# FordyceLab/magnify

Hardware: AMD Instinct MI355X
Metric: megapixels/sec through flatfield+segment+ROI-reduce; markers/sec (higher is better)
Workload: dtype u16

## Files before the change

magnify_amd/csrc/mg_edges.hip:

```cpp
#include <math.h>
#include <stdlib.h>

#include <algorithm>

#include "mg_common.h"

namespace {

constexpr int TW = 256;
constexpr int TH = 64;
constexpr int NT = 256;
constexpr int RPW = 16;
constexpr int LPAD = 16;
constexpr int LS = TW + 2 * LPAD;
constexpr int CHUNKS = LS / 16;

struct U8Scale {
  double mn, top, scale, offset;
  int passthrough;
};

__device__ __forceinline__ U8Scale make_scale(const double* d_minmax, int plane) {
  U8Scale s;
  s.passthrough = (d_minmax == nullptr);
// ... 551 lines not shown
}

__device__ __forceinline__ int nth_window(const int32_t* coarse, int p) {
  int last = -1;
  for (int it = 0; it <= p; ++it) {
    int best = 0x7FFFFFFF;
#pragma unroll
    for (int k = 0; k < 4; ++k)
      if (coarse[k] > last && coarse[k] < best) best = coarse[k];
    if (best == 0x7FFFFFFF) return -1;
    last = best;
  }
  return last;
}

__device__ __forceinline__ long long block_exscan_i64(long long mine, long long* s_pre) {
  s_pre[threadIdx.x] = mine;
  __syncthreads();
  for (int off = 1; off < NT; off <<= 1) {
    const long long v = (int)threadIdx.x >= off ? s_pre[threadIdx.x - off] : 0;
    __syncthreads();
    s_pre[threadIdx.x] += v;
    __syncthreads();
  }
  return s_pre[threadIdx.x] - mine;
}

__global__ __launch_bounds__(NT) void k_edge_thresholds(const uint32_t* __restrict__ d_hist, int n_fine, int n_bins,
                                                        long long r0, long long r1, long long r2, long long r3,
                                                        float gamma_lo, float gamma_hi, int32_t* __restrict__ d_thresh,
                                                        float* __restrict__ d_quantiles, int32_t* __restrict__ d_unresolved,
                                                        int32_t* __restrict__ d_state, uint32_t* __restrict__ d_win_base) {
  __shared__ int s_bin[4];
  __shared__ long long s_below[4];
  __shared__ uint32_t s_hist[FINE + COARSE];
  const int plane = blockIdx.x;
  const uint32_t* hist_g = d_hist + (int64_t)plane * n_bins;
  for (int i = threadIdx.x; i < n_bins; i += NT) s_hist[i] = hist_g[i];
  __syncthreads();
  const uint32_t* hist = s_hist;
  const int per = (n_bins + NT - 1) / NT;
  const int b0 = threadIdx.x * per, b1 = min(b0 + per, n_bins);
  long long mine = 0;
  for (int b = b0; b < b1; ++b) mine += hist[b];
  __shared__ long long s_pre[NT];
  long long run = block_exscan_i64(mine, s_pre);
  if (threadIdx.x < 4) s_bin[threadIdx.x] = n_bins, s_below[threadIdx.x] = 0;
  __syncthreads();
  const long long ranks[4] = {r0, r1, r2, r3};
  for (int b = b0; b < b1; ++b) {
    const long long nxt = run + hist[b];
#pragma unroll
    for (int k = 0; k < 4; ++k)
      if (run <= ranks[k] && ranks[k] < nxt) s_bin[k] = b, s_below[k] = run;
    run = nxt;
  }
  __syncthreads();
  if (threadIdx.x == 0) {
    int32_t order[4], coarse[4];
#pragma unroll
    for (int k = 0; k < 4; ++k) {
      const bool fine = s_bin[k] < n_fine || s_bin[k] >= n_bins;
      order[k] = fine ? s_bin[k] : 0;
      coarse[k] = fine ? -1 : s_bin[k] - n_fine;
    }
    int n_win = 0;
    while (nth_window(coarse, n_win) >= 0) ++n_win;
    d_unresolved[plane] = n_win | (n_win << 8);
    if (d_state) {
      int32_t* st = d_state + (int64_t)plane * TS_WORDS;
#pragma unroll
      for (int k = 0; k < 4; ++k) {
        st[TS_ORDER + k] = order[k];
        st[TS_COARSE + k] = coarse[k];
        st[TS_RESID + k] = (int32_t)(ranks[k] - s_below[k]);
      }
      st[TS_NWIN] = n_win;
    }
    if (d_win_base) d_win_base[plane] = n_win > 0 ? (uint32_t)nth_window(coarse, 0) << 13 : MG_HIST_SKIP;
    finish_thresholds(order, gamma_lo, gamma_hi, plane, d_thresh, d_quantiles);
  }
}

__global__ __launch_bounds__(NT) void k_window_resolve(const uint32_t* __restrict__ d_hist_win, int pass, float gamma_lo,
                                                       float gamma_hi, int32_t* __restrict__ d_state,
                                                       uint32_t* __restrict__ d_win_base, int32_t* __restrict__ d_thresh,
                                                       float* __restrict__ d_quantiles, int32_t* __restrict__ d_unresolved) {
  __shared__ int s_pos[4];
  __shared__ long long s_pre[NT];
  const int plane = blockIdx.x;
  int32_t* st = d_state + (int64_t)plane * TS_WORDS;
  const int n_win = st[TS_NWIN];
  if (pass >= n_win) return;
  int32_t coarse[4], resid[4];
#pragma unroll
  for (int k = 0; k < 4; ++k) coarse[k] = st[TS_COARSE + k], resid[k] = st[TS_RESID + k];
  const int cbin = nth_window(coarse, pass);
  const uint32_t* hist = d_hist_win + (int64_t)plane * FINE;
  constexpr int PER = FINE / NT;
  uint32_t mine_v[PER];
  long long mine = 0;
#pragma unroll
  for (int j = 0; j < PER; ++j) mine_v[j] = hist[threadIdx.x * PER + j], mine += mine_v[j];
  long long run = block_exscan_i64(mine, s_pre);
  if (threadIdx.x < 4) s_pos[threadIdx.x] = 0;
  __syncthreads();
#pragma unroll
  for (int j = 0; j < PER; ++j) {
    const long long nxt = run + mine_v[j];
#pragma unroll
    for (int k = 0; k < 4; ++k)
      if (coarse[k] == cbin && run <= (long long)resid[k] && (long long)resid[k] < nxt) s_pos[k] = threadIdx.x * PER + j;
    run = nxt;
  }
  __syncthreads();
  if (threadIdx.x == 0) {
    int32_t order[4];
#pragma unroll
    for (int k = 0; k < 4; ++k) {
      order[k] = st[TS_ORDER + k];
      if (coarse[k] == cbin) order[k] = (cbin << 13) + s_pos[k], st[TS_ORDER + k] = order[k];
    }
    const int left = n_win - 1 - pass;
    d_unresolved[plane] = left | (n_win << 8);
    d_win_base[plane] = left > 0 ? (uint32_t)nth_window(coarse, pass + 1) << 13 : MG_HIST_SKIP;
    if (left == 0) finish_thresholds(order, gamma_lo, gamma_hi, plane, d_thresh, d_quantiles);
  }
}

__device__ __forceinline__ uint32_t bits_at(const uint32_t* __restrict__ bits, int64_t bit0, int n) {
  const int64_t wi = bit0 >> 5;
  const int sh = (int)(bit0 & 31);
  uint64_t two = bits[wi];
  if (sh + n > 32) two |= (uint64_t)bits[wi + 1] << 32;
  const uint32_t v = (uint32_t)(two >> sh);
  return n >= 32 ? v : (v & ((1u << n) - 1u));
}
__device__ __forceinline__ void bits_or(uint32_t* __restrict__ bits, int64_t bit0, uint32_t v) {
  if (!v) return;
  const int64_t wi = bit0 >> 5;
  const int sh = (int)(bit0 & 31);
  atomicOr(&bits[wi], v << sh);
  if (sh && (v >> (32 - sh))) atomicOr(&bits[wi + 1], v >> (32 - sh));
}
__device__ __forceinline__ uint32_t row_word(const uint32_t* __restrict__ bits, int h, int w, int y, int x0) {
  if (y < 0 || y >= h) return 0u;
  const int lo = max(x0, 0), hi = min(x0 + 32, w);
  if (lo >= hi) return 0u;
  return bits_at(bits, (int64_t)y * w + lo, hi - lo) << (lo - x0);
}

__device__ __forceinline__ uint32_t shl1_or(uint32_t v, uint64_t mask) {
  uint32_t out;
  uint64_t carry_out;
  asm("v_addc_co_u32_e64 %0, %1, %2, %2, %3" : "=v"(out), "=s"(carry_out) : "v"(v), "s"(mask));
  return out;
}

__device__ __forceinline__ uint32_t or_reduce8(uint32_t v) {
  v |= (uint32_t)__builtin_amdgcn_update_dpp(0, (int)v, 0xB1, 0xF, 0xF, true);
  v |= (uint32_t)__builtin_amdgcn_update_dpp(0, (int)v, 0x4E, 0xF, 0xF, true);
  v |= (uint32_t)__builtin_amdgcn_update_dpp(0, (int)v, 0x141, 0xF, 0xF, true);
  return v;
}

__global__ __launch_bounds__(NT) void k_canny_nms(const uint8_t* __restrict__ d_blur, int h, int w,
                                                  const int32_t* __restrict__ d_thresh, int64_t words_per_plane,
                                                  uint32_t* __restrict__ d_weak, uint32_t* __restrict__ d_strong,
                                                  uint32_t* __restrict__ d_class) {
  __shared__ __attribute__((aligned(16))) uint8_t tile[TH + 4][LS];
  const int plane = blockIdx.z;
  const int tx0 = blockIdx.x * TW, ty0 = blockIdx.y * TH;
  U8Scale sc;
  sc.passthrough = 1;
  load_tile<uint8_t, 2>(d_blur + (int64_t)plane * h * w, w, h, w, tx0, ty0, sc, tile);
  __syncthreads();
  const int low = d_thresh[2 * plane], high = d_thresh[2 * plane + 1];
  const int lane = threadIdx.x & 63, wave = threadIdx.x >> 6;
  const int c0 = 4 * lane, gx = tx0 + c0;
  uint32_t* weak = d_weak + plane * words_per_plane;
  uint32_t* strong = d_strong + plane * words_per_plane;
  uint32_t* cls0 = d_class ? d_class + (3 * plane) * words_per_plane : nullptr;
  uint32_t* cls1 = d_class ? d_class + (3 * plane + 1) * words_per_plane : nullptr;
  uint32_t* cls2 = d_class ? d_class + (3 * plane + 2) * words_per_plane : nullptr;
  constexpr int TG22 = 13573;
  const uint32_t in_row = gx + 4 <= w ? 0xFu : ((1u << max(w - gx, 0)) - 1u);
  typedef short s2 __attribute__((ext_vector_type(2)));
  typedef unsigned short u2 __attribute__((ext_vector_type(2)));
  struct Pairs4 {
    u2 p[4];
  };
  auto unpack = [](const Row12& r) {
    Pairs4 o;
    o.p[0] = __builtin_bit_cast(u2, __builtin_amdgcn_perm(0u, r.d0, 0x0C030C02u));
    o.p[1] = __builtin_bit_cast(u2, __builtin_amdgcn_perm(0u, r.d1, 0x0C010C00u));
    o.p[2] = __builtin_bit_cast(u2, __builtin_amdgcn_perm(0u, r.d1, 0x0C030C02u));
    o.p[3] = __builtin_bit_cast(u2, __builtin_amdgcn_perm(0u, r.d2, 0x0C010C00u));
    return o;
  };
  int mg[3][6];
  uint32_t cxy[2][4];
  Pairs4 ua = unpack(read_row(tile, wave * RPW, c0)), ub = unpack(read_row(tile, wave * RPW + 1, c0));
#pragma unroll
  for (int jr = 2; jr < RPW + 4; ++jr) {
    const Pairs4 uc = unpack(read_row(tile, wave * RPW + jr, c0));
    const int ym = ty0 - 2 + wave * RPW + jr - 1;
#pragma unroll
    for (int k = 0; k < 6; ++k) mg[0][k] = mg[1][k], mg[1][k] = mg[2][k];
#pragma unroll
    for (int q = 0; q < 4; ++q) cxy[0][q] = cxy[1][q];
    {
      s2 S[4], D[4];
#pragma unroll
      for (int k = 0; k < 4; ++k) {
        S[k] = __builtin_bit_cast(s2, (u2)((ua.p[k] + uc.p[k]) * (unsigned short)3 + ub.p[k] * (unsigned short)10));
        D[k] = __builtin_bit_cast(s2, uc.p[k]) - __builtin_bit_cast(s2, ua.p[k]);
      }
      uint32_t xy[6];
#pragma unroll
      for (int jp = 0; jp < 3; ++jp) {
        const s2 dxp = S[jp + 1] - S[jp];
        const s2 mid = __builtin_bit_cast(s2, __builtin_amdgcn_alignbit(__builtin_bit_cast(uint32_t, D[jp + 1]),
                                                                         __builtin_bit_cast(uint32_t, D[jp]), 16));
        const s2 dyp = (D[jp] + D[jp + 1]) * (short)3 + mid * (short)10;
        xy[2 * jp] = __builtin_amdgcn_perm(__builtin_bit_cast(uint32_t, dyp), __builtin_bit_cast(uint32_t, dxp), 0x05040100u);
        xy[2 * jp + 1] = __builtin_amdgcn_perm(__builtin_bit_cast(uint32_t, dyp), __builtin_bit_cast(uint32_t, dxp), 0x07060302u);
      }
      const bool row_in = ym >= 0 && ym < h;
#pragma unroll
      for (int k = 0; k < 6; ++k) {
        const int x = gx + k - 1;
        const int m = __builtin_amdgcn_sdot2(__builtin_bit_cast(s2, xy[k]), __builtin_bit_cast(s2, xy[k]), 0, false);
        mg[2][k] = (row_in && x >= 0 && x < w) ? m : 0;
        if (k >= 1 && k <= 4) cxy[1][k - 1] = xy[k];
      }
    }
    ua = ub;
    ub = uc;
    if (jr < 4) continue;
    const int yo = ym - 1;
    uint32_t wb = 0, sb = 0, cb0 = 0, cb1 = 0, cb2 = 0;
    if (yo < h) {
#pragma unroll
      for (int q = 3; q >= 0; --q) {
        const int m = mg[1][q + 1];
        const int xs = (int)(int16_t)(cxy[0][q] & 0xFFFFu), ys = (int)cxy[0][q] >> 16;
        const int x = abs(xs), ay = abs(ys), y = ay << 15;
        const int tg22x = x * TG22;
        const int tg67x = tg22x + (x << 16);
        const uint64_t horiz = __ballot(y < tg22x);
        const uint64_t vert = __ballot(y > tg67x) & ~horiz;
        const bool neg_b = (xs ^ ys) < 0;
        const uint64_t neg = __ballot(neg_b);
        const uint64_t ok_h = __ballot(m > mg[1][q]) & __ballot(m >= mg[1][q + 2]);
        const uint64_t ok_v = __ballot(m > mg[0][q + 1]) & __ballot(m >= mg[2][q + 1]);
        const uint64_t ok_d = __ballot(m > mg[0][q]) & __ballot(m > mg[2][q + 2]);
        const uint64_t ok_n = __ballot(m > mg[0][q + 2]) & __ballot(m > mg[2][q]);
        const uint64_t is_max = (horiz & ok_h) | (vert & ok_v) | (~(horiz | vert) & ((neg & ok_n) | (~neg & ok_d)));
        const uint64_t cand = is_max & __ballot(m > low) & __ballot(gx + q < w);
        wb = shl1_or(wb, cand);
        sb = shl1_or(sb, cand & __ballot(m > high));
        const bool le_b = ay <= x, ge_b = ay >= x;
        const uint64_t le = __ballot(le_b), ge = __ballot(ge_b);
        cb0 = shl1_or(cb0, (neg & le) | (~neg & ge));
        cb1 = shl1_or(cb1, neg);
        const bool lowq = neg_b ? le_b : !ge_b;
        const int sq = lowq ? x + ay : ay - x;
        const uint64_t upper = __ballot(sq * sq > 2 * x * x);
        cb2 = shl1_or(cb2, neg ^ upper);
      }
    }
    wb = or_reduce8(wb << (4 * (lane & 7)));
    sb = or_reduce8(sb << (4 * (lane & 7)));
    if (d_class) {
      cb0 = or_reduce8((cb0 & in_row) << (4 * (lane & 7)));
      cb1 = or_reduce8((cb1 & in_row) << (4 * (lane & 7)));
      cb2 = or_reduce8((cb2 & in_row) << (4 * (lane & 7)));
    }
    if ((lane & 7) == 0 && yo < h && gx < w) {
      const int64_t bit0 = (int64_t)yo * w + gx;
      if ((bit0 & 31) == 0 && gx + 32 <= w) {
        weak[bit0 >> 5] = wb;
        strong[bit0 >> 5] = sb;
        if (d_class) {
          cls0[bit0 >> 5] = cb0;
          cls1[bit0 >> 5] = cb1;
          cls2[bit0 >> 5] = cb2;
        }
      } else {
        bits_or(weak, bit0, wb);
        bits_or(strong, bit0, sb);
        if (d_class) {
          bits_or(cls0, bit0, cb0);
          bits_or(cls1, bit0, cb1);
          bits_or(cls2, bit0, cb2);
        }
      }
    }
  }
}

constexpr int HW = TW / 32;
constexpr int HTH = 256;

__device__ __forceinline__ uint32_t lds_interior(const uint32_t (*a)[HW + 2], int r, int k) {
  return (r >= 1 && r <= HTH && k >= 1 && k <= HW) ? a[r][k] : 0u;
}

__global__ __launch_bounds__(NT) void k_hysteresis(const uint32_t* __restrict__ d_weak, uint32_t* __restrict__ d_strong,
                                                   int64_t words_per_plane, int h, int w,
                                                   uint32_t* __restrict__ d_changed,
                                                   const uint8_t* __restrict__ d_flags_in,
                                                   uint8_t* __restrict__ d_flags_out) {
  __shared__ uint32_t st[HTH + 2][HW + 2];
  __shared__ uint32_t wk[HTH + 2][HW + 2];
  __shared__ uint32_t s_mark;
  const int plane = blockIdx.z;
  const int tx0 = blockIdx.x * TW, ty0 = blockIdx.y * HTH;
  const int ntx = gridDim.x, nty = gridDim.y;
  if (d_flags_in && !d_flags_in[(int64_t)plane * ntx * nty + blockIdx.y * ntx + blockIdx.x]) return;
  const uint32_t* weak = d_weak + plane * words_per_plane;
  uint32_t* strong = d_strong + plane * words_per_plane;
  int pending = 0;
  if ((w & 31) == 0) {
    constexpr int TOTAL = (HTH + 2) * (HW + 2), ITER = (TOTAL + NT - 1) / NT;
    uint32_t sv[ITER], wv[ITER];
#pragma unroll
    for (int it = 0; it < ITER; ++it) {
      const int i = min((int)threadIdx.x + it * NT, TOTAL - 1);
      const int r = i / (HW + 2), kk = i - r * (HW + 2);
      const int y = ty0 - 1 + r, x = tx0 - 32 + 32 * kk;
      const bool in = y >= 0 && y < h && x >= 0 && x < w;
      const int64_t wi = in ? ((int64_t)y * w + x) >> 5 : 0;
      sv[it] = strong[wi];
      wv[it] = weak[wi];
      if (!in) sv[it] = 0u, wv[it] = 0u;
    }
#pragma unroll
    for (int it = 0; it < ITER; ++it) {
      const int i = threadIdx.x + it * NT;
      if (i < TOTAL) {
        const int r = i / (HW + 2), kk = i - r * (HW + 2);
        st[r][kk] = sv[it];
        wk[r][kk] = wv[it];
        if (r >= 1 && r <= HTH && kk >= 1 && kk <= HW) pending |= (wv[it] & ~sv[it]) != 0;
      }
    }
  } else {
    for (int i = threadIdx.x; i < (HTH + 2) * (HW + 2); i += NT) {
      const int r = i / (HW + 2), kk = i - r * (HW + 2);
      const uint32_t sv = row_word(strong, h, w, ty0 - 1 + r, tx0 - 32 + 32 * kk);
      const uint32_t wv = row_word(weak, h, w, ty0 - 1 + r, tx0 - 32 + 32 * kk);
      st[r][kk] = sv;
      wk[r][kk] = wv;
      if (r >= 1 && r <= HTH && kk >= 1 && kk <= HW) pending |= (wv & ~sv) != 0;
    }
  }
  if (threadIdx.x == 0) s_mark = 0u;
  if (!__syncthreads_or(pending)) return;
  constexpr int WPT = HTH * HW / NT;
  static_assert(WPT * NT == HTH * HW, "the tile's words must divide evenly over the threads");
  const int k = (threadIdx.x & (HW - 1)) + 1, r0 = WPT * (threadIdx.x / HW) + 1;
  uint32_t first[WPT];
#pragma unroll
  for (int j = 0; j < WPT; ++j) first[j] = st[r0 + j][k];
  int again;
  do {
    int changed = 0;
#pragma unroll
    for (int j = 0; j < WPT; ++j) {
      const int r = r0 + j;
      uint32_t cur = st[r][k];
      uint32_t cand = wk[r][k] & ~cur;
      if (!cand) continue;
      uint32_t dil = 0;
#pragma unroll
      for (int dr = -1; dr <= 1; ++dr) {
        const uint32_t c = st[r + dr][k], l = st[r + dr][k - 1], rt = st[r + dr][k + 1];
        dil |= c | (c << 1) | (c >> 1) | (l >> 31) | (rt << 31);
      }
      uint32_t nw = cand & dil;
      if (!nw) continue;
      cur |= nw;
      cand &= ~nw;
      for (uint32_t g = cand & ((cur << 1) | (cur >> 1)); g; g = cand & ((cur << 1) | (cur >> 1))) {
        cur |= g;
        cand &= ~g;
      }
      st[r][k] = cur;
      changed = 1;
    }
    again = __syncthreads_or(changed);
  } while (again);
#pragma unroll
  for (int j = 0; j < WPT; ++j) {
    const uint32_t diff = st[r0 + j][k] & ~first[j];
    wk[r0 + j][k] = diff;
    if (diff) bits_or(strong, (int64_t)(ty0 + r0 + j - 1) * w + tx0 + 32 * (k - 1), diff);
  }
  __syncthreads();
  for (int i = threadIdx.x; i < 2 * (HW + 2) + 2 * HTH; i += NT) {
    int r, kk;
    if (i < HW + 2) r = 0, kk = i;
    else if (i < 2 * (HW + 2)) r = HTH + 1, kk = i - (HW + 2);
    else if (i < 2 * (HW + 2) + HTH) r = i - 2 * (HW + 2) + 1, kk = 0;
    else r = i - 2 * (HW + 2) - HTH + 1, kk = HW + 1;
    const uint32_t cand = wk[r][kk] & ~st[r][kk];
    if (!cand) continue;
    uint32_t dil = 0;
#pragma unroll
    for (int dr = -1; dr <= 1; ++dr) {
      const uint32_t c = lds_interior(wk, r + dr, kk), l = lds_interior(wk, r + dr, kk - 1), rt = lds_interior(wk, r + dr, kk + 1);
      dil |= c | (c << 1) | (c >> 1) | (l >> 31) | (rt << 31);
    }
    if (cand & dil) {
      const int dy = r == 0 ? -1 : (r == HTH + 1 ? 1 : 0), dx = kk == 0 ? -1 : (kk == HW + 1 ? 1 : 0);
      atomicOr(&s_mark, 1u << ((dy + 1) * 3 + dx + 1));
    }
  }
  __syncthreads();
  if (threadIdx.x == 0 && s_mark) {
    const uint32_t m = s_mark;
    bool any = false;
    for (int d = 0; d < 9; ++d) {
      if (!((m >> d) & 1u)) continue;
      const int nx = (int)blockIdx.x + d % 3 - 1, ny = (int)blockIdx.y + d / 3 - 1;
      if (nx < 0 || nx >= ntx || ny < 0 || ny >= nty) continue;
      any = true;
      if (d_flags_out) d_flags_out[(int64_t)plane * ntx * nty + ny * ntx + nx] = 1;
    }
    if (any && __hip_atomic_load(&d_changed[plane], __ATOMIC_RELAXED, __HIP_MEMORY_SCOPE_AGENT) == 0u) d_changed[plane] = 1u;
  }
}

__global__ __launch_bounds__(NT) void k_unpack_bits(const uint32_t* __restrict__ d_bits, int64_t words_per_plane,
                                                    int64_t npix, uint8_t* __restrict__ d_out) {
  const int plane = blockIdx.y;
  const uint32_t* bits = d_bits + plane * words_per_plane;
  for (int64_t i = (int64_t)blockIdx.x * NT + threadIdx.x; i < npix; i += (int64_t)gridDim.x * NT)
    d_out[plane * npix + i] = (bits[i >> 5] >> (i & 31)) & 1u;
}

__device__ __forceinline__ uint32_t bits_at_nb(const uint32_t* __restrict__ bits, int64_t bit0, int n) {
  const int64_t wi = bit0 >> 5;
  const int sh = (int)(bit0 & 31);
  const uint64_t two = (uint64_t)bits[wi] | ((uint64_t)bits[wi + 1] << 32);
  const uint32_t v = (uint32_t)(two >> sh);
  return n >= 32 ? v : (v & ((1u << n) - 1u));
}

__global__ __launch_bounds__(NT) void k_cell_count(const uint32_t* __restrict__ d_bits, int64_t words_per_plane, int h,
                                                   int w, int grid, int gc, int n_cells,
                                                   int32_t* __restrict__ d_counts, unsigned long long* __restrict__ d_state,
                                                   int state_words) {
  const int plane = blockIdx.y;
  const int cell = blockIdx.x * NT + threadIdx.x;
  if (d_state && cell < state_words) d_state[(int64_t)plane * state_words + cell] = 0ull;
  if (cell >= n_cells) return;
  const uint32_t* bits = d_bits + plane * words_per_plane;
  const int cr = cell / gc, cc = cell - cr * gc;
  const int y0 = cr * grid, x0 = cc * grid;
  const int ch = min(grid, h - y0), cw = min(grid, w - x0);
  int cnt = 0;
#pragma unroll 5
  for (int r = 0; r < ch; ++r)
    for (int c0 = 0; c0 < cw; c0 += 32)
      cnt += __popc(bits_at_nb(bits, (int64_t)(y0 + r) * w + x0 + c0, min(32, cw - c0)));
  d_counts[(int64_t)plane * n_cells + cell] = cnt;
}

__device__ __forceinline__ void put_edge_count(int plane, int total, int64_t limit, int32_t* d_num_edges, int32_t* d_totals) {
  if (d_totals) d_totals[plane] = total;
  d_num_edges[plane] = (limit >= 0 && total > limit) ? 0 : total;
}

__global__ __launch_bounds__(1024) void k_cell_scan(const int32_t* __restrict__ d_counts, int n_cells,
                                                    int32_t* __restrict__ d_starts, int32_t* __restrict__ d_num_edges,
                                                    int32_t* __restrict__ d_totals, int64_t limit) {
  const int plane = blockIdx.x;
  const int32_t* cnt = d_counts + (int64_t)plane * n_cells;
  int32_t* st = d_starts + (int64_t)plane * n_cells;
  const int per = (n_cells + 1023) / 1024;
  const int lo = min((int)threadIdx.x * per, n_cells), hi = min(lo + per, n_cells);
  int sum = 0;
  for (int i = lo; i < hi; ++i) sum += cnt[i];
  int total;
  int run = mg_block_exscan(sum, &total);
  for (int i = lo; i < hi; ++i) {
    st[i] = run;
    run += cnt[i];
  }
  if (threadIdx.x == 0) put_edge_count(plane, total, limit, d_num_edges, d_totals);
}

constexpr int SCAN_CHUNK = 4096;

__global__ __launch_bounds__(1024) void k_cell_scan_chunks(const int32_t* __restrict__ d_counts, int n_cells,
                                                           int32_t* __restrict__ d_starts, int32_t* __restrict__ d_num_edges,
                                                           int32_t* __restrict__ d_totals, int64_t limit,
                                                           unsigned long long* __restrict__ d_state) {
  const int plane = blockIdx.y, n_chunks = gridDim.x;
  const int32_t* cnt = d_counts + (int64_t)plane * n_cells;
  int32_t* st = d_starts + (int64_t)plane * n_cells;
  unsigned long long* state = d_state + (int64_t)plane * (n_chunks + 1);
  __shared__ int s_chunk;
  if (threadIdx.x == 0) s_chunk = (int)atomicAdd(&state[n_chunks], 1ull);
  __syncthreads();
  const int chunk = s_chunk;
  const int i0 = chunk * SCAN_CHUNK + 4 * (int)threadIdx.x;
  int c[4] = {0, 0, 0, 0};
  const bool vec = (n_cells & 3) == 0 && i0 + 4 <= n_cells;
  if (vec) {
    const int4 v = *reinterpret_cast<const int4*>(cnt + i0);
    c[0] = v.x, c[1] = v.y, c[2] = v.z, c[3] = v.w;
  } else {
#pragma unroll
    for (int j = 0; j < 4; ++j)
      if (i0 + j < n_cells) c[j] = cnt[i0 + j];
  }
  int total;
  int run = mg_block_exscan(c[0] + c[1] + c[2] + c[3], &total);
  __shared__ int s_base;
  if (threadIdx.x == 0)
    __hip_atomic_store(&state[chunk], (1ull << 63) | (uint32_t)total, __ATOMIC_RELEASE, __HIP_MEMORY_SCOPE_AGENT);
  if (threadIdx.x < 64) {
    int base = 0;
    for (int j = threadIdx.x; j < chunk; j += 64) {
      unsigned long long v;
      do {
        v = __hip_atomic_load(&state[j], __ATOMIC_ACQUIRE, __HIP_MEMORY_SCOPE_AGENT);
      } while (!(v >> 63));
      base += (int)(uint32_t)v;
    }
#pragma unroll
    for (int off = 32; off > 0; off >>= 1) base += __shfl_xor(base, off);
    if (threadIdx.x == 0) s_base = base;
  }
  __syncthreads();
  run += s_base;
  if (vec) {
    *reinterpret_cast<int4*>(st + i0) = make_int4(run, run + c[0], run + c[0] + c[1], run + c[0] + c[1] + c[2]);
  } else {
#pragma unroll
    for (int j = 0; j < 4; ++j) {
      if (i0 + j < n_cells) st[i0 + j] = run;
      run += c[j];
    }
  }
  if (chunk == n_chunks - 1 && threadIdx.x == 0) put_edge_count(plane, s_base + total, limit, d_num_edges, d_totals);
}

__global__ __launch_bounds__(NT) void k_cell_fill(const uint32_t* __restrict__ d_bits, int64_t words_per_plane, int h,
                                                  int w, int grid, int gc, int n_cells,
                                                  const int32_t* __restrict__ d_starts, int32_t* __restrict__ d_coords,
                                                  int64_t coord_cap) {
  const int plane = blockIdx.y;
  const int cell = blockIdx.x * NT + threadIdx.x;
  if (cell >= n_cells) return;
  const uint32_t* bits = d_bits + plane * words_per_plane;
  const int cr = cell / gc, cc = cell - cr * gc;
  const int y0 = cr * grid, x0 = cc * grid;
  const int ch = min(grid, h - y0), cw = min(grid, w - x0);
  int2* out = reinterpret_cast<int2*>(d_coords + (int64_t)plane * coord_cap * 2);
  int64_t pos = d_starts[(int64_t)plane * n_cells + cell];
  for (int r = 0; r < ch; ++r)
    for (int c0 = 0; c0 < cw; c0 += 32) {
      uint32_t v = bits_at(bits, (int64_t)(y0 + r) * w + x0 + c0, min(32, cw - c0));
      while (v) {
        const int b = __ffs(v) - 1;
        v &= v - 1;
        if (pos < coord_cap) out[pos] = make_int2(y0 + r, x0 + c0 + b);
        ++pos;
      }
    }
}

constexpr int FILL_TRIPS = 4;

__global__ __launch_bounds__(NT) void k_cell_fill_rows(const uint32_t* __restrict__ d_bits, int64_t words_per_plane,
                                                       int h, int w, int grid, int gc, int n_cells,
                                                       const int32_t* __restrict__ d_starts,
                                                       int32_t* __restrict__ d_coords, int64_t coord_cap) {
  const int plane = blockIdx.y;
  const int cpw = 64 / grid;
  const int lane = threadIdx.x & 63;
  const int64_t wave = ((int64_t)blockIdx.x * NT + threadIdx.x) >> 6;
  const int ci = lane / grid, r = lane - ci * grid;
  const uint32_t* bits = d_bits + plane * words_per_plane;
  uint64_t rowbits[FILL_TRIPS];
  int y[FILL_TRIPS], x0[FILL_TRIPS];
  int64_t pos[FILL_TRIPS];
#pragma unroll
  for (int q = 0; q < FILL_TRIPS; ++q) {
    const int64_t cell = (wave * FILL_TRIPS + q) * cpw + ci;
    rowbits[q] = 0, y[q] = 0, x0[q] = 0, pos[q] = 0;
    if (ci < cpw && cell < n_cells) {
      const int cr = (int)(cell / gc), cc = (int)(cell - (int64_t)cr * gc);
      y[q] = cr * grid + r;
      x0[q] = cc * grid;
      const int cw = min(grid, w - x0[q]);
      if (y[q] < h) {
        const int64_t b0 = (int64_t)y[q] * w + x0[q];
        rowbits[q] = bits_at_nb(bits, b0, min(32, cw));
        if (cw > 32) rowbits[q] |= (uint64_t)bits_at_nb(bits, b0 + 32, cw - 32) << 32;
      }
      pos[q] = d_starts[(int64_t)plane * n_cells + cell];
    }
  }
  constexpr int CH = 512;
  __shared__ int2 s_stage[NT / 64][CH];
  int2* stage = s_stage[threadIdx.x >> 6];
  int2* out = reinterpret_cast<int2*>(d_coords + (int64_t)plane * coord_cap * 2);
#pragma unroll
  for (int q = 0; q < FILL_TRIPS; ++q) {
    const int cnt = __popcll(rowbits[q]);
    const int incl = mg_wave_scan_incl_i32(cnt);
    const int total = __shfl(incl, 63);
    const int lpos = incl - cnt;
    const int64_t base = __shfl(pos[q], 0);
    const bool any_cell = (wave * FILL_TRIPS + q) * cpw < n_cells;
    for (int c0 = 0; c0 < total; c0 += CH) {
      uint64_t rb = rowbits[q];
      int li = lpos - c0;
      while (rb) {
        const int b = __ffsll((unsigned long long)rb) - 1;
        rb &= rb - 1;
        if (li >= 0 && li < CH) stage[li] = make_int2(y[q], x0[q] + b);
        ++li;
      }
      __builtin_amdgcn_fence(__ATOMIC_SEQ_CST, "wavefront");
      const int n = min(total - c0, CH);
      for (int i = lane; i < n; i += 64) {
        const int64_t p = base + c0 + i;
        if (any_cell && p < coord_cap) out[p] = stage[i];
      }
      __builtin_amdgcn_fence(__ATOMIC_SEQ_CST, "wavefront");
    }
  }
}

__global__ __launch_bounds__(NT) void k_edge_angles(const uint8_t* __restrict__ d_blur, int h, int w,
                                                    const int32_t* __restrict__ d_coords, int64_t coord_cap,
                                                    const int32_t* __restrict__ d_num_edges,
                                                    float* __restrict__ d_angle) {
  const int plane = blockIdx.y;
  const int n = min((int64_t)d_num_edges[plane], coord_cap);
  const uint8_t* pb = d_blur + (int64_t)plane * h * w;
  const int2* co = reinterpret_cast<const int2*>(d_coords + (int64_t)plane * coord_cap * 2);
  float* pa = d_angle + (int64_t)plane * h * w;
  for (int64_t i = (int64_t)blockIdx.x * NT + threadIdx.x; i < n; i += (int64_t)gridDim.x * NT) {
    const int2 yx = co[i];
    pa[(int64_t)yx.x * w + yx.y] = mg_edge_angle(pb, h, w, yx.x, yx.y);
  }
}

inline dim3 tile_grid(int h, int w, int n_planes) { return dim3((w + TW - 1) / TW, (h + TH - 1) / TH, n_planes); }
inline bool words_ok(int64_t words_per_plane, int h, int w) {
  return words_per_plane * 32 >= (((int64_t)h * w + 31) / 32) * 32 + 32;
}

}

extern "C" int mg_to_uint8_blur(const void* d_src, int dtype, int n_planes, int64_t plane_stride, int h, int w,
                                int64_t row_stride, const double* d_minmax, uint8_t* d_blur, uint8_t* d_u8,
                                void* stream) {
  if (!d_src || !d_blur || n_planes < 0 || h < 0 || w < 0) return MG_EINVAL;
  if (!d_minmax && dtype != MG_U8) return MG_EINVAL;
  if (n_planes == 0 || h == 0 || w == 0) return MG_OK;
  const dim3 g = tile_grid(h, w, n_planes);
  if (g.y > 65535 || g.z > 65535) return MG_EINVAL;
  hipStream_t s = mg_stream(stream);
  return mg_dispatch_pixel(dtype, [&](auto t) {
    using T = decltype(t);
    hipLaunchKernelGGL((k_u8_blur<T>), g, dim3(NT), 0, s, (const T*)d_src, plane_stride, h, w, row_stride, d_minmax,
                       d_blur, d_u8);
    MG_CHECK_LAUNCH();
    return MG_OK;
  });
}

extern "C" int64_t mg_scharr_hist_scratch_words(int n_planes, int h, int w, int mode) {
  if (n_planes < 0 || h < 0 || w < 0 || (mode != 0 && mode != 1)) return -1;
  const dim3 t = tile_grid(h, w, n_planes);
  const int64_t slots = (int64_t)t.x * ((t.y + HIST_TILES - 1) / HIST_TILES);
  return (int64_t)n_planes * slots * ((mode == 0 ? FINE + COARSE : FINE) / 2);
}

extern "C" int mg_scharr_hist(const uint8_t* d_blur, int n_planes, int h, int w, int mode, const uint32_t* d_base,
                              uint32_t* d_hist, uint32_t* d_scratch, int64_t scratch_words, void* stream) {
  if (!d_blur || !d_hist || n_planes < 0 || h < 0 || w < 0 || (mode != 0 && mode != 1)) return MG_EINVAL;
  if (mode == 1 && !d_base) return MG_EINVAL;
  if (n_planes == 0 || h == 0 || w == 0) return MG_OK;
  const dim3 t = tile_grid(h, w, n_planes);
  const dim3 g(t.x, (t.y + HIST_TILES - 1) / HIST_TILES, t.z);
  if (g.y > 65535 || g.z > 65535) return MG_EINVAL;
  if (d_scratch && scratch_words < mg_scharr_hist_scratch_words(n_planes, h, w, mode)) return MG_EINVAL;
  const int n_bins = mode == 0 ? FINE + COARSE : FINE;
  const size_t lds = (size_t)(TH + 2) * LS + (size_t)n_bins * 2;
  static bool attr_set = false;
  if (!attr_set) {
    if (hipFuncSetAttribute(reinterpret_cast<const void*>(k_scharr_hist<false>),
                            hipFuncAttributeMaxDynamicSharedMemorySize, 96 * 1024) != hipSuccess)
      return MG_ELAUNCH;
    attr_set = true;
  }
  const int split = d_scratch ? 1 : 0;
  if (split) {
    hipLaunchKernelGGL(k_scharr_hist<true>, g, dim3(NT), (size_t)n_bins * 2, mg_stream(stream), d_blur, h, w, mode,
                       d_base, n_bins, d_hist, d_scratch, split);
    MG_CHECK_LAUNCH();
  }
  hipLaunchKernelGGL(k_scharr_hist<false>, t, dim3(NT), lds, mg_stream(stream), d_blur, h, w, mode, d_base, n_bins,
                     d_hist, d_scratch, split);
  MG_CHECK_LAUNCH();
  if (d_scratch) {
    const int slots = (int)(g.x * g.y);
    hipLaunchKernelGGL(k_hist_reduce, dim3((n_bins / 2 + NT - 1) / NT, n_planes, (slots + HIST_SLOTS_PER_BLOCK - 1) / HIST_SLOTS_PER_BLOCK),
                       dim3(NT), 0, mg_stream(stream), d_scratch, slots, n_bins, d_hist, mode == 1 ? d_base : nullptr);
    MG_CHECK_LAUNCH();
  }
  return MG_OK;
}

static bool blur_hist_fused(const void* d_src, int dtype, int64_t plane_stride, int h, int w, int64_t row_stride,
                            const uint8_t* d_blur, const uint8_t* d_u8) {
  if (d_u8 || (dtype != MG_U8 && dtype != MG_U16) || h < 2 || w < 8 || (w & 3)) return false;
  const int64_t esz = dtype == MG_U8 ? 1 : 2;
  return (reinterpret_cast<uintptr_t>(d_src) % (4 * esz)) == 0 && plane_stride % 4 == 0 && row_stride % 4 == 0 &&
         (reinterpret_cast<uintptr_t>(d_blur) & 3) == 0;
}

extern "C" int64_t mg_blur_hist_scratch_words(int n_planes, int h, int w) {
  if (n_planes < 0 || h < 0 || w < 0) return -1;
  const int64_t fused = (int64_t)n_planes * ((w + FW - 1) / FW) * ((h + FH - 1) / FH) * ((FINE + COARSE) / 2);
  return std::max(fused, mg_scharr_hist_scratch_words(n_planes, h, w, 0));
}

extern "C" int mg_to_uint8_blur_hist(const void* d_src, int dtype, int n_planes, int64_t plane_stride, int h, int w,
                                     int64_t row_stride, const double* d_minmax, uint8_t* d_blur, uint8_t* d_u8,
                                     uint32_t* d_hist, uint32_t* d_scratch, int64_t scratch_words, void* stream) {
  if (!d_src || !d_blur || !d_hist || n_planes < 0 || h < 0 || w < 0) return MG_EINVAL;
  if (!d_minmax && dtype != MG_U8) return MG_EINVAL;
  if (n_planes == 0 || h == 0 || w == 0) return MG_OK;
  if (d_scratch && scratch_words < mg_blur_hist_scratch_words(n_planes, h, w)) return MG_EINVAL;
  static const bool off = getenv("MG_NO_BLUR_HIST") != nullptr;
  if (off || !d_scratch || !blur_hist_fused(d_src, dtype, plane_stride, h, w, row_stride, d_blur, d_u8)) {
    const int rc = mg_to_uint8_blur(d_src, dtype, n_planes, plane_stride, h, w, row_stride, d_minmax, d_blur, d_u8, stream);
    if (rc != MG_OK) return rc;
    return mg_scharr_hist(d_blur, n_planes, h, w, 0, nullptr, d_hist, d_scratch, scratch_words, stream);
  }
  const dim3 g((w + FW - 1) / FW, (h + FH - 1) / FH, n_planes);
  if (g.y > 65535 || g.z > 65535) return MG_EINVAL;
  hipStream_t s = mg_stream(stream);
  constexpr int n_bins = FINE + COARSE;
  if (dtype == MG_U8)
    hipLaunchKernelGGL((k_blur_hist<uint8_t>), g, dim3(NT), (size_t)n_bins * 2, s, (const uint8_t*)d_src, plane_stride, h, w,
                       row_stride, d_minmax, d_blur, d_scratch);
  else
    hipLaunchKernelGGL((k_blur_hist<uint16_t>), g, dim3(NT), (size_t)n_bins * 2, s, (const uint16_t*)d_src, plane_stride, h,
                       w, row_stride, d_minmax, d_blur, d_scratch);
  MG_CHECK_LAUNCH();
  const int slots = (int)(g.x * g.y);
  hipLaunchKernelGGL(k_hist_reduce, dim3((n_bins / 2 + NT - 1) / NT, n_planes, (slots + HIST_SLOTS_PER_BLOCK - 1) / HIST_SLOTS_PER_BLOCK),
                     dim3(NT), 0, s, d_scratch, slots, n_bins, d_hist, (const uint32_t*)nullptr);
  MG_CHECK_LAUNCH();
  return MG_OK;
}

extern "C" int mg_edge_thresholds(const uint32_t* d_hist, int n_planes, const int64_t* ranks4, float gamma_low,
                                  float gamma_high, int32_t* d_thresh, float* d_quantiles, int32_t* d_unresolved,
                                  int32_t* d_state, uint32_t* d_win_base, void* stream) {
  if (!d_hist || !ranks4 || !d_thresh || !d_quantiles || !d_unresolved || n_planes < 0) return MG_EINVAL;
  if ((d_state == nullptr) != (d_win_base == nullptr)) return MG_EINVAL;
  if (n_planes == 0) return MG_OK;
  hipLaunchKernelGGL(k_edge_thresholds, dim3(n_planes), dim3(NT), 0, mg_stream(stream), d_hist, FINE, FINE + COARSE,
                     (long long)ranks4[0], (long long)ranks4[1], (long long)ranks4[2], (long long)ranks4[3], gamma_low,
                     gamma_high, d_thresh, d_quantiles, d_unresolved, d_state, d_win_base);
  MG_CHECK_LAUNCH();
  return MG_OK;
}

extern "C" int mg_edge_thresholds_window(const uint32_t* d_hist_win, int n_planes, int pass, float gamma_low,
                                         float gamma_high, int32_t* d_state, uint32_t* d_win_base, int32_t* d_thresh,
                                         float* d_quantiles, int32_t* d_unresolved, void* stream) {
  if (!d_hist_win || !d_state || !d_win_base || !d_thresh || !d_quantiles || !d_unresolved || n_planes < 0 || pass < 0 ||
      pass > 3)
    return MG_EINVAL;
  if (n_planes == 0) return MG_OK;
  hipLaunchKernelGGL(k_window_resolve, dim3(n_planes), dim3(NT), 0, mg_stream(stream), d_hist_win, pass, gamma_low,
                     gamma_high, d_state, d_win_base, d_thresh, d_quantiles, d_unresolved);
  MG_CHECK_LAUNCH();
  return MG_OK;
}

extern "C" int mg_canny_nms(const uint8_t* d_blur, int n_planes, int h, int w, const int32_t* d_thresh,
                            uint32_t* d_weak, uint32_t* d_strong, uint32_t* d_class, int64_t words_per_plane,
                            void* stream) {
  if (!d_blur || !d_thresh || !d_weak || !d_strong || n_planes < 0 || h < 0 || w < 0) return MG_EINVAL;
  if (n_planes == 0 || h == 0 || w == 0) return MG_OK;
  if (!words_ok(words_per_plane, h, w)) return MG_EINVAL;
  const dim3 g = tile_grid(h, w, n_planes);
  if (g.y > 65535 || g.z > 65535) return MG_EINVAL;
  hipStream_t s = mg_stream(stream);
  const size_t bytes = (size_t)n_planes * words_per_plane * 4;
  if ((w & 31) && (mg_zero_async(d_weak, bytes, s) != hipSuccess || mg_zero_async(d_strong, bytes, s) != hipSuccess ||
                   (d_class && mg_zero_async(d_class, 3 * bytes, s) != hipSuccess)))
    return MG_ELAUNCH;
  hipLaunchKernelGGL(k_canny_nms, g, dim3(NT), 0, s, d_blur, h, w, d_thresh, words_per_plane, d_weak, d_strong,
                     d_class);
  MG_CHECK_LAUNCH();
  return MG_OK;
}

extern "C" int mg_canny_hysteresis(const uint32_t* d_weak, uint32_t* d_strong, int64_t words_per_plane, int n_planes,
                                   int h, int w, uint32_t* d_changed, const uint8_t* d_flags_in, uint8_t* d_flags_out,
                                   void* stream) {
  if (!d_weak || !d_strong || !d_changed || n_planes < 0 || h < 0 || w < 0) return MG_EINVAL;
  if (n_planes == 0 || h == 0 || w == 0) return MG_OK;
  if (!words_ok(words_per_plane, h, w)) return MG_EINVAL;
  const dim3 g((w + TW - 1) / TW, (h + HTH - 1) / HTH, n_planes);
  if (g.y > 65535 || g.z > 65535) return MG_EINVAL;
  hipLaunchKernelGGL(k_hysteresis, g, dim3(NT), 0, mg_stream(stream), d_weak, d_strong, words_per_plane, h, w,
                     d_changed, d_flags_in, d_flags_out);
  MG_CHECK_LAUNCH();
  return MG_OK;
}

extern "C" int mg_hysteresis_tiles(int h, int w, int* tiles_x, int* tiles_y) {
  if (!tiles_x || !tiles_y) return MG_EINVAL;
  *tiles_x = (w + TW - 1) / TW;
  *tiles_y = (h + HTH - 1) / HTH;
  return MG_OK;
}

extern "C" int mg_unpack_bits(const uint32_t* d_bits, int64_t words_per_plane, int n_planes, int64_t n_bits,
                              uint8_t* d_out, void* stream) {
  if (!d_bits || !d_out || n_planes < 0 || n_planes > 65535 || n_bits < 0 || words_per_plane * 32 < n_bits)
    return MG_EINVAL;
  if (n_planes == 0 || n_bits == 0) return MG_OK;
  const int bx = (int)std::min<int64_t>((n_bits + NT - 1) / NT, 4096);
  hipLaunchKernelGGL(k_unpack_bits, dim3(bx, n_planes), dim3(NT), 0, mg_stream(stream), d_bits, words_per_plane, n_bits,
                     d_out);
  MG_CHECK_LAUNCH();
  return MG_OK;
}

extern "C" int64_t mg_edge_grid_scan_words(int n_planes, int h, int w, int grid) {
  if (n_planes < 0 || h < 0 || w < 0 || grid <= 0) return -1;
  const int64_t n_cells = (int64_t)((h + grid - 1) / grid) * ((w + grid - 1) / grid);
  return (int64_t)n_planes * ((n_cells + SCAN_CHUNK - 1) / SCAN_CHUNK + 1);
}

extern "C" int mg_edge_grid(const uint32_t* d_edge_bits, int64_t words_per_plane, int n_planes, int h, int w, int grid,
                            int32_t* d_cell_counts, int32_t* d_cell_starts, int32_t* d_num_edges, int32_t* d_coords,
                            int64_t coord_cap, uint64_t* d_scan_state, int32_t* d_edge_totals, int phases, void* stream) {
  if (!d_edge_bits || !d_cell_counts || !d_cell_starts || !d_num_edges || n_planes < 0 || grid <= 0 || coord_cap < 0 ||
      n_planes > 65535 || phases < 1 || phases > 3 || ((phases & 2) && !d_coords))
    return MG_EINVAL;
  if (n_planes == 0) return MG_OK;
  if (!words_ok(words_per_plane, h, w)) return MG_EINVAL;
  const int gr = (h + grid - 1) / grid, gc = (w + grid - 1) / grid, n_cells = gr * gc;
  hipStream_t s = mg_stream(stream);
  if (phases & 1) {
    const int n_chunks = (n_cells + SCAN_CHUNK - 1) / SCAN_CHUNK;
    const bool chunked = d_scan_state && n_chunks > 1 && n_chunks <= 65535 && n_chunks + 1 <= n_cells;
    if (n_cells > 0) {
      hipLaunchKernelGGL(k_cell_count, dim3((n_cells + NT - 1) / NT, n_planes), dim3(NT), 0, s, d_edge_bits,
                         words_per_plane, h, w, grid, gc, n_cells, d_cell_counts,
                         chunked ? reinterpret_cast<unsigned long long*>(d_scan_state) : nullptr, n_chunks + 1);
      MG_CHECK_LAUNCH();
    }
    const int64_t limit = (phases & 2) ? coord_cap : -1;
    if (chunked) {
      hipLaunchKernelGGL(k_cell_scan_chunks, dim3(n_chunks, n_planes), dim3(1024), 0, s, d_cell_counts, n_cells,
                         d_cell_starts, d_num_edges, d_edge_totals, limit, reinterpret_cast<unsigned long long*>(d_scan_state));
    } else {
      hipLaunchKernelGGL(k_cell_scan, dim3(n_planes), dim3(1024), 0, s, d_cell_counts, n_cells, d_cell_starts, d_num_edges,
                         d_edge_totals, limit);
    }
    MG_CHECK_LAUNCH();
  }
  if ((phases & 2) && n_cells > 0) {
    if (grid <= 64) {
      const int64_t groups = (n_cells + 64 / grid - 1) / (64 / grid);
      const int64_t waves = (groups + FILL_TRIPS - 1) / FILL_TRIPS;
      hipLaunchKernelGGL(k_cell_fill_rows, dim3((unsigned)((waves + NT / 64 - 1) / (NT / 64)), n_planes), dim3(NT), 0, s,
                         d_edge_bits, words_per_plane, h, w, grid, gc, n_cells, d_cell_starts, d_coords, coord_cap);
    } else {
      hipLaunchKernelGGL(k_cell_fill, dim3((n_cells + NT - 1) / NT, n_planes), dim3(NT), 0, s, d_edge_bits,
                         words_per_plane, h, w, grid, gc, n_cells, d_cell_starts, d_coords, coord_cap);
    }
    MG_CHECK_LAUNCH();
  }
  return MG_OK;
}

extern "C" int mg_edge_angles(const uint8_t* d_blur, int n_planes, int h, int w, const int32_t* d_coords,
                              int64_t coord_cap, const int32_t* d_num_edges, float* d_angle, void* stream) {
  if (!d_blur || !d_coords || !d_num_edges || !d_angle || n_planes < 0 || n_planes > 65535 || coord_cap < 0)
    return MG_EINVAL;
  if (n_planes == 0 || coord_cap == 0) return MG_OK;
  const int bx = (int)std::max<int64_t>(1, std::min<int64_t>((coord_cap + NT - 1) / NT, 1 << 20));
  hipLaunchKernelGGL(k_edge_angles, dim3(bx, n_planes), dim3(NT), 0, mg_stream(stream), d_blur, h, w, d_coords,
                     coord_cap, d_num_edges, d_angle);
  MG_CHECK_LAUNCH();
  return MG_OK;
}
```

Measured before the change: 213,200.

## Compact hysteresis launches to flagged tiles with per-block tile chunks

Adds a hysteresis kernel variant in which each block reads 32 tile flags, ballots the active ones, and loops over only the flagged tiles. The old full-grid kernel remains for the first pass (no input flags) or when an environment override is set. The aim is to stop launching and retiring many blocks that exit at once in later iterations, where few tiles are active. The trade-off is that flagged tiles sharing a chunk now run one after another inside one block, which cuts parallelism when many tiles are active; there is also a getenv call on every launch.

```diff
diff --git a/magnify_amd/csrc/mg_edges.hip b/magnify_amd/csrc/mg_edges.hip
--- a/magnify_amd/csrc/mg_edges.hip
+++ b/magnify_amd/csrc/mg_edges.hip
@@ -877,23 +877,26 @@
 
 constexpr int HW = TW / 32;
 constexpr int HTH = 256;
+constexpr int HYST_CHUNK = 32;
+static_assert(HYST_CHUNK <= NT, "one flag byte per thread");
 
 __device__ __forceinline__ uint32_t lds_interior(const uint32_t (*a)[HW + 2], int r, int k) {
   return (r >= 1 && r <= HTH && k >= 1 && k <= HW) ? a[r][k] : 0u;
 }
 
-__global__ __launch_bounds__(NT) void k_hysteresis(const uint32_t* __restrict__ d_weak, uint32_t* __restrict__ d_strong,
-                                                   int64_t words_per_plane, int h, int w,
-                                                   uint32_t* __restrict__ d_changed,
-                                                   const uint8_t* __restrict__ d_flags_in,
-                                                   uint8_t* __restrict__ d_flags_out) {
-  __shared__ uint32_t st[HTH + 2][HW + 2];
-  __shared__ uint32_t wk[HTH + 2][HW + 2];
-  __shared__ uint32_t s_mark;
-  const int plane = blockIdx.z;
-  const int tx0 = blockIdx.x * TW, ty0 = blockIdx.y * HTH;
-  const int ntx = gridDim.x, nty = gridDim.y;
-  if (d_flags_in && !d_flags_in[(int64_t)plane * ntx * nty + blockIdx.y * ntx + blockIdx.x]) return;
+struct HystLds {
+  uint32_t st[HTH + 2][HW + 2];
+  uint32_t wk[HTH + 2][HW + 2];
+  uint32_t mark;
+};
+
+__device__ __forceinline__ void hysteresis_tile(HystLds& lds, const uint32_t* __restrict__ d_weak,
+                                                uint32_t* __restrict__ d_strong, int64_t words_per_plane, int h, int w,
+                                                uint32_t* __restrict__ d_changed, uint8_t* __restrict__ d_flags_out,
+                                                int plane, int tile_x, int tile_y, int ntx, int nty) {
+  uint32_t (*st)[HW + 2] = lds.st;
+  uint32_t (*wk)[HW + 2] = lds.wk;
+  const int tx0 = tile_x * TW, ty0 = tile_y * HTH;
   const uint32_t* weak = d_weak + plane * words_per_plane;
   uint32_t* strong = d_strong + plane * words_per_plane;
   int pending = 0;
@@ -931,7 +934,7 @@
       if (r >= 1 && r <= HTH && kk >= 1 && kk <= HW) pending |= (wv & ~sv) != 0;
     }
   }
-  if (threadIdx.x == 0) s_mark = 0u;
+  if (threadIdx.x == 0) lds.mark = 0u;
   if (!__syncthreads_or(pending)) return;
   constexpr int WPT = HTH * HW / NT;
   static_assert(WPT * NT == HTH * HW, "the tile's words must divide evenly over the threads");
@@ -990,21 +993,59 @@
     }
     if (cand & dil) {
       const int dy = r == 0 ? -1 : (r == HTH + 1 ? 1 : 0), dx = kk == 0 ? -1 : (kk == HW + 1 ? 1 : 0);
-      atomicOr(&s_mark, 1u << ((dy + 1) * 3 + dx + 1));
+      atomicOr(&lds.mark, 1u << ((dy + 1) * 3 + dx + 1));
     }
   }
   __syncthreads();
-  if (threadIdx.x == 0 && s_mark) {
-    const uint32_t m = s_mark;
+  if (threadIdx.x == 0 && lds.mark) {
+    const uint32_t m = lds.mark;
     bool any = false;
     for (int d = 0; d < 9; ++d) {
       if (!((m >> d) & 1u)) continue;
-      const int nx = (int)blockIdx.x + d % 3 - 1, ny = (int)blockIdx.y + d / 3 - 1;
+      const int nx = tile_x + d % 3 - 1, ny = tile_y + d / 3 - 1;
       if (nx < 0 || nx >= ntx || ny < 0 || ny >= nty) continue;
       any = true;
       if (d_flags_out) d_flags_out[(int64_t)plane * ntx * nty + ny * ntx + nx] = 1;
     }
     if (any && __hip_atomic_load(&d_changed[plane], __ATOMIC_RELAXED, __HIP_MEMORY_SCOPE_AGENT) == 0u) d_changed[plane] = 1u;
+  }
+}
+
+__global__ __launch_bounds__(NT) void k_hysteresis(const uint32_t* __restrict__ d_weak, uint32_t* __restrict__ d_strong,
+                                                   int64_t words_per_plane, int h, int w,
+                                                   uint32_t* __restrict__ d_changed,
+                                                   const uint8_t* __restrict__ d_flags_in,
+                                                   uint8_t* __restrict__ d_flags_out) {
+  __shared__ HystLds lds;
+  const int plane = blockIdx.z, ntx = gridDim.x, nty = gridDim.y;
+  if (d_flags_in && !d_flags_in[(int64_t)plane * ntx * nty + blockIdx.y * ntx + blockIdx.x]) return;
+  hysteresis_tile(lds, d_weak, d_strong, words_per_plane, h, w, d_changed, d_flags_out, plane, blockIdx.x, blockIdx.y, ntx,
+                  nty);
+}
+
+__global__ __launch_bounds__(NT) void k_hysteresis_asked(const uint32_t* __restrict__ d_weak, uint32_t* __restrict__ d_strong,
+                                                         int64_t words_per_plane, int h, int w, int ntx, int nty,
+                                                         uint32_t* __restrict__ d_changed,
+                                                         const uint8_t* __restrict__ d_flags_in,
+                                                         uint8_t* __restrict__ d_flags_out) {
+  __shared__ HystLds lds;
+  constexpr int WAVES = (HYST_CHUNK + 63) / 64;
+  __shared__ unsigned long long s_asked[WAVES];
+  const int plane = blockIdx.y, n_tiles = ntx * nty;
+  const int t0 = blockIdx.x * HYST_CHUNK, t = t0 + (int)threadIdx.x;
+  const bool asked = (int)threadIdx.x < HYST_CHUNK && t < n_tiles && d_flags_in[(int64_t)plane * n_tiles + t] != 0;
+  const unsigned long long mine = __ballot(asked);
+  if ((threadIdx.x & 63) == 0 && threadIdx.x < 64 * WAVES) s_asked[threadIdx.x >> 6] = mine;
+  __syncthreads();
+  for (int wv = 0; wv < WAVES; ++wv) {
+    const unsigned long long all = s_asked[wv];
+    unsigned long long m = (unsigned long long)__builtin_amdgcn_readfirstlane((uint32_t)all) |
+                           ((unsigned long long)__builtin_amdgcn_readfirstlane((uint32_t)(all >> 32)) << 32);
+    for (; m; m &= m - 1) {
+      const int tile = t0 + 64 * wv + __ffsll((long long)m) - 1;
+      hysteresis_tile(lds, d_weak, d_strong, words_per_plane, h, w, d_changed, d_flags_out, plane, tile % ntx, tile / ntx,
+                      ntx, nty);
+    }
   }
 }
 
@@ -1395,8 +1436,17 @@
   if (!words_ok(words_per_plane, h, w)) return MG_EINVAL;
   const dim3 g((w + TW - 1) / TW, (h + HTH - 1) / HTH, n_planes);
   if (g.y > 65535 || g.z > 65535) return MG_EINVAL;
-  hipLaunchKernelGGL(k_hysteresis, g, dim3(NT), 0, mg_stream(stream), d_weak, d_strong, words_per_plane, h, w,
-                     d_changed, d_flags_in, d_flags_out);
+  const char* env = getenv("MG_HYST_FULL_GRID");
+  if (!d_flags_in || (env && env[0] == '1')) {
+    hipLaunchKernelGGL(k_hysteresis, g, dim3(NT), 0, mg_stream(stream), d_weak, d_strong, words_per_plane, h, w,
+                       d_changed, d_flags_in, d_flags_out);
+  } else {
+    const int64_t n_tiles = (int64_t)g.x * g.y;
+    if (n_tiles > INT32_MAX) return MG_EINVAL;
+    hipLaunchKernelGGL(k_hysteresis_asked, dim3((unsigned)((n_tiles + HYST_CHUNK - 1) / HYST_CHUNK), n_planes),
+                       dim3(NT), 0, mg_stream(stream), d_weak, d_strong, words_per_plane, h, w, (int)g.x, (int)g.y, d_changed,
+                       d_flags_in, d_flags_out);
+  }
   MG_CHECK_LAUNCH();
   return MG_OK;
 }
```

Result: slower. 206,500 (-3.1%).
